# kdexd/virtex

Measured on NVIDIA H100. Metric: image-caption pairs/sec bicaptioning R50-L1-H1024, higher is better.
Workload: dtype bf16

## Files before the change

virtex_b200/csrc/gemm_tc.cu:

```cuda
#include <stdlib.h>
#include "ptx.cuh"
#include "vtx_common.cuh"
#include "../../include/virtex_b200.h"

#define KP_TAPS_W p.taps_w
#define KP_PAD p.pad
#define KP_NTAPS p.ntaps

namespace vtx {

constexpr int kBM = 128;
constexpr int kBK = 64;
constexpr int kMaxStages = 8;
constexpr int kABytes = kBM * kBK * 2;
constexpr int kSmemTotal = 232448;
constexpr int kCtrlBytes = 1024;
constexpr int kThreads = 384;
constexpr int kEpiThreads = 256;

struct FastDiv {
  uint32_t mul, shr;
};
__device__ __forceinline__ int fdiv(int x, const FastDiv& f) {
  return f.mul == 0u ? x : (int)(__umulhi((uint32_t)x, f.mul) >> f.shr);
// ... 684 lines not shown
      }
      if (bnr_on) {
        const uint32_t cp = smem_u32(cbuf) + (scg >> 3) * 16384 + bnr_r0 * 128;
        const int c8 = scg & 7;
        float mean[8], sc[8], sh[8];
        {
          const float4 m0 = __ldg(reinterpret_cast<const float4*>(p.bnr_bnp + bnr_col));
          const float4 m1 = __ldg(reinterpret_cast<const float4*>(p.bnr_bnp + bnr_col + 4));
          mean[0] = m0.x; mean[1] = m0.y; mean[2] = m0.z; mean[3] = m0.w;
          mean[4] = m1.x; mean[5] = m1.y; mean[6] = m1.z; mean[7] = m1.w;
          const float4 a0 = __ldg(reinterpret_cast<const float4*>(p.bnr_bnp + 2 * p.N + bnr_col));
          const float4 a1 = __ldg(reinterpret_cast<const float4*>(p.bnr_bnp + 2 * p.N + bnr_col + 4));
          const float4 b0 = __ldg(reinterpret_cast<const float4*>(p.bnr_bnp + 3 * p.N + bnr_col));
          const float4 b1 = __ldg(reinterpret_cast<const float4*>(p.bnr_bnp + 3 * p.N + bnr_col + 4));
          sc[0] = a0.x; sc[1] = a0.y; sc[2] = a0.z; sc[3] = a0.w; sc[4] = a1.x; sc[5] = a1.y; sc[6] = a1.z; sc[7] = a1.w;
          sh[0] = b0.x; sh[1] = b0.y; sh[2] = b0.z; sh[3] = b0.w; sh[4] = b1.x; sh[5] = b1.y; sh[6] = b1.z; sh[7] = b1.w;
        }
        for (int rb = 0; rb < st_rpt; rb += 4) {
          uint4 yv[4];
          uint32_t mbits;
          bnr_load(rb, yv, mbits);
#pragma unroll
          for (int r4 = 0; r4 < 4; ++r4) {
            const int r = rb + r4;
            const uint4 raw = lds128(cp + r * 128 + ((c8 ^ ((bnr_r0 + r) & 7)) << 4));
            float f[8], yy[8];
            unpack8(*reinterpret_cast<const bf16x8*>(&raw), f);
            unpack8(*reinterpret_cast<const bf16x8*>(&yv[r4]), yy);
#pragma unroll
            for (int i = 0; i < 8; ++i) {
              const bool on = p.bnr == 1 ? ((yy[i] * sc[i] + sh[i] > 0.f) && ((mbits >> (8 * r4)) & 0xffu) != 0u)
                                         : (((mbits >> (8 * r4 + i)) & 1u) != 0u);
              const float dz = on ? f[i] : 0.f;
              st_s[i] += dz;
              st_q[i] += dz * (yy[i] - mean[i]);
            }
          }
        }
      }
      if (!p.bnr && p.stats != nullptr && st_on) {
        const int r0 = srg * st_rpt;
        const uint32_t cp = smem_u32(cbuf) + (scg >> 3) * 16384 + r0 * 128;
        const int c8 = scg & 7;
        for (int rb = 0; rb < st_rpt; rb += 4) {
#pragma unroll
          for (int r4 = 0; r4 < 4; ++r4) {
            const int r = rb + r4;
            const uint4 raw = lds128(cp + r * 128 + ((c8 ^ ((r0 + r) & 7)) << 4));
            float f[8];
            unpack8(*reinterpret_cast<const bf16x8*>(&raw), f);
#pragma unroll
            for (int i = 0; i < 8; ++i) {
              st_s[i] += f[i];
              st_q[i] += f[i] * f[i];
            }
          }
        }
      }
    }
  }
  if (staged) {
    if (et == 0) tma_store_wait_read<0>();
    epi_bar(bar_id, epi_threads);
    if (p.stats != nullptr && st_nt >= 0) flush_stats(cstage0 + (PP ? (size_t)wg * p.cbytes : 0));
  }
}

typedef CUresult (*PFN_encodeTiled)(CUtensorMap*, CUtensorMapDataType, cuuint32_t, void*, const cuuint64_t*,
                                    const cuuint64_t*, const cuuint32_t*, const cuuint32_t*, CUtensorMapInterleave,
                                    CUtensorMapSwizzle, CUtensorMapL2promotion, CUtensorMapFloatOOBfill);

static PFN_encodeTiled get_encode() {
  static PFN_encodeTiled fn = nullptr;
  if (fn == nullptr) {
    void* p = nullptr;
    cudaDriverEntryPointQueryResult q;
    if (cudaGetDriverEntryPoint("cuTensorMapEncodeTiled", &p, cudaEnableDefault, &q) == cudaSuccess &&
        q == cudaDriverEntryPointSuccess)
      fn = reinterpret_cast<PFN_encodeTiled>(p);
  }
  return fn;
}

static int make_tmap(CUtensorMap* tm, const void* ptr, int rank, const uint64_t* dims, const uint64_t* strides_elems,
                     const uint32_t* box, const uint32_t* estr = nullptr) {
  PFN_encodeTiled enc = get_encode();
  if (!enc) return set_error(VTX_ECUDA, "cuTensorMapEncodeTiled entry point not available");
  cuuint64_t gdim[5];
  cuuint64_t gstr[5];
  cuuint32_t bx[5];
  cuuint32_t es[5];
  for (int i = 0; i < rank; ++i) {
    gdim[i] = dims[i];
    bx[i] = box[i];
    es[i] = estr ? estr[i] : 1;
  }
  for (int i = 0; i < rank - 1; ++i) gstr[i] = strides_elems[i] * 2;
  if ((reinterpret_cast<uintptr_t>(ptr) & 15) != 0) return set_error(VTX_EINVAL, "TMA base pointer not 16B aligned");
  for (int i = 0; i < rank - 1; ++i)
    if (gstr[i] % 16 != 0) return set_error(VTX_EINVAL, "TMA stride not a multiple of 16 bytes");
  CUresult r = enc(tm, CU_TENSOR_MAP_DATA_TYPE_BFLOAT16, (cuuint32_t)rank, const_cast<void*>(ptr), gdim, gstr, bx, es,
                   CU_TENSOR_MAP_INTERLEAVE_NONE, CU_TENSOR_MAP_SWIZZLE_128B, CU_TENSOR_MAP_L2_PROMOTION_L2_256B,
                   CU_TENSOR_MAP_FLOAT_OOB_FILL_NONE);
  if (r != CUDA_SUCCESS) return set_error(VTX_ECUDA, "cuTensorMapEncodeTiled failed (%d)", (int)r);
  return VTX_OK;
}

constexpr int kSchedSlots = 4096;
static int g_sched_dynamic = 0;
static struct SchedRing {
  unsigned int* ctr;
  unsigned int base[kSchedSlots];
  unsigned int next;
} g_sched[64];
static bool sched_is_dynamic() {
  static const char* env = getenv("VTX_GEMM_SCHEDULE");
  return env != nullptr ? (env[0] == 'd') : (g_sched_dynamic != 0);
}
static unsigned int* sched_slot(unsigned int fetches, unsigned int* base_out) {
  if (!sched_is_dynamic()) return nullptr;
  int dev = 0;
  cudaGetDevice(&dev);
  if (dev < 0 || dev >= 64) return nullptr;
  SchedRing& r = g_sched[dev];
  if (r.ctr == nullptr) {
    unsigned int* ptr = nullptr;
    if (cudaMalloc(&ptr, sizeof(unsigned int) * kSchedSlots) != cudaSuccess) return nullptr;
    cudaMemset(ptr, 0, sizeof(unsigned int) * kSchedSlots);
    cudaDeviceSynchronize();
    memset(r.base, 0, sizeof(r.base));
    r.next = 0;
    r.ctr = ptr;
  }
  const unsigned int slot = r.next++ % kSchedSlots;
  *base_out = r.base[slot];
  r.base[slot] += fetches;
  return r.ctr + slot;
}

static int ilog2(int x) {
  int l = 0;
  while ((1 << l) < x) ++l;
  return l;
}

static void choose_box(int H, int W, int positions, int* bw, int* bh, int* bn) {
  int best_w = 1, best_h = 1;
  double best_eff = -1;
  for (int w = 1; w <= positions; w <<= 1)
    for (int h = 1; w * h <= positions; h <<= 1) {
      if (w > 2 * W || h > 2 * H) continue;
      const int tw = (W + w - 1) / w, th = (H + h - 1) / h;
      const double eff = (double)(W * H) / ((double)tw * w * th * h);
      const double score = eff * 1000.0 + w * 0.01 + h * 0.0001;
      if (score > best_eff) { best_eff = score; best_w = w; best_h = h; }
    }
  *bw = best_w; *bh = best_h; *bn = positions / (best_w * best_h);
}

template <bool SS>
static cudaError_t launch_gemm(const cudaLaunchConfig_t& cfg, bool pingpong, int bn, const CUtensorMap& tmA,
                               const CUtensorMap& tmB, const CUtensorMap& tmD, const CUtensorMap& tmR,
                               const CUtensorMap& tmY, const GemmKParams& p) {
  if (pingpong && bn == 64) return cudaLaunchKernelEx(&cfg, gemm_wgmma_kernel<64, true, SS>, tmA, tmB, tmD, tmR, tmY, p);
  if (pingpong) return cudaLaunchKernelEx(&cfg, gemm_wgmma_kernel<128, true, SS>, tmA, tmB, tmD, tmR, tmY, p);
  if (bn == 64) return cudaLaunchKernelEx(&cfg, gemm_wgmma_kernel<64, false, SS>, tmA, tmB, tmD, tmR, tmY, p);
  if (bn == 128) return cudaLaunchKernelEx(&cfg, gemm_wgmma_kernel<128, false, SS>, tmA, tmB, tmD, tmR, tmY, p);
  if (bn == 192) return cudaLaunchKernelEx(&cfg, gemm_wgmma_kernel<192, false, SS>, tmA, tmB, tmD, tmR, tmY, p);
  return cudaLaunchKernelEx(&cfg, gemm_wgmma_kernel<256, false, SS>, tmA, tmB, tmD, tmR, tmY, p);
}

bool resid_dgrad_serves(const VtxGemm* g);
int resid_dgrad(const VtxGemm* g, cudaStream_t stream);

}

using namespace vtx;

extern "C" int vtx_gemm_set_dynamic_schedule(int on) {
  g_sched_dynamic = on ? 1 : 0;
  return VTX_OK;
}

extern "C" int vtx_gemm(const VtxGemm* g, void* stream_) {
  cudaStream_t stream = reinterpret_cast<cudaStream_t>(stream_);
  if (!g || !g->A || !g->B || !g->D) return set_error(VTX_EINVAL, "vtx_gemm: null pointer");
  if (g->M <= 0 || g->N <= 0 || g->K <= 0) return set_error(VTX_EINVAL, "vtx_gemm: empty problem");
  if (g->atomic && !g->out_f32) return set_error(VTX_EINVAL, "vtx_gemm: atomic accumulate needs fp32 output");
  if (g->split_k > 1 && !g->atomic) return set_error(VTX_EINVAL, "vtx_gemm: split_k > 1 needs atomic = 1");
  if (g->stats && (g->out_f32 || g->bias || g->residual || g->act || (g->alpha != 0.f && g->alpha != 1.f)))
    return set_error(VTX_EINVAL, "vtx_gemm: stats needs a plain bf16 output (no bias/residual/activation/alpha)");
  if (g->ldd % (g->out_f32 ? 4 : 8) != 0) return set_error(VTX_EINVAL, "vtx_gemm: ldd must keep rows 16B aligned");
  if (g->conv_mode < 0 || g->conv_mode > 6 || g->conv_mode == 3)
    return set_error(VTX_EINVAL, "vtx_gemm: conv_mode must be 0, 1, 2, 4, 5 or 6");
  VtxGemm g4;
  const bool trans_d = g->conv_mode == 4;
  if (trans_d) {
    if (g->conv_c != 64 || g->N != 64 || g->M != 9 * 64 || !g->out_f32 || !g->atomic)
      return set_error(VTX_EINVAL, "vtx_gemm: conv_mode 4 needs C = Cout = 64, M = 576, fp32 atomic output");
    g4 = *g;
    g4.conv_mode = 2;
    g4.M = g->N;
    g4.N = g->M;
    g4.split_k = vtx_num_sms() / 3;
    g4.conv_stride = 1;
    g4.conv_taps = 0;
    g = &g4;
  }
  const int split_k = g->split_k > 1 ? g->split_k : 1;

  GemmKParams p;
  memset(&p, 0, sizeof(p));
  p.M = g->M; p.N = g->N; p.K = g->K;
  p.a_mn = g->a_mn; p.b_mn = g->b_mn;
  p.mode = g->conv_mode;
  const bool stem = g->conv_mode == 5 || g->conv_mode == 6;
  p.taps_w = 3; p.pad = 1; p.ntaps = 9;
  if (stem) { p.mode = g->conv_mode == 5 ? 1 : 2; p.taps_w = 1; p.pad = 0; p.ntaps = 4; }
  const bool one_tap = !stem && g->conv_taps == 1;
  if (one_tap) { p.taps_w = 1; p.pad = 0; p.ntaps = 1; }
  const bool tap_grid = !stem && !one_tap && g->conv_taps_h > 0;
  if (tap_grid) {
    if (p.mode != 1 || g->conv_taps_w <= 0 || g->conv_taps_h > 3 || g->conv_taps_w > 3 || g->conv_pad < 0 || g->conv_pad > 1)
      return set_error(VTX_EINVAL, "vtx_gemm: bad explicit tap grid");
    p.taps_w = g->conv_taps_w; p.pad = g->conv_pad; p.ntaps = g->conv_taps_h * g->conv_taps_w;
  }
  const int cstride = (g->conv_stride == 2 && (p.mode == 1 || p.mode == 2) && !stem) ? 2 : 1;
  if (g->conv_stride != 0 && g->conv_stride != 1 && cstride != 2)
    return set_error(VTX_EINVAL, "vtx_gemm: conv_stride 2 is supported for conv_mode 1 / 2 only");
  if (g->conv_taps != 0 && g->conv_taps != 1 && g->conv_taps != 9) return set_error(VTX_EINVAL, "vtx_gemm: conv_taps must be 0, 1 or 9");
  p.cstride = cstride;
  const int ntaps = stem ? 4 : one_tap ? 1 : tap_grid ? p.ntaps : 9;
  if (p.mode == 1) { p.a_mn = 0; p.b_mn = 0; }
  if (p.mode == 2) { p.a_mn = 1; p.b_mn = 1; }
  int bn = g->tile_n;
  if (bn == 0) {
    const int gran = p.b_mn ? 64 : 16;
    if (g->N >= 256) bn = 256;
    else bn = ((g->N + gran - 1) / gran) * gran;
    if (bn == 256 && split_k == 1) {
      const long mt = (g->M + kBM - 1) / kBM;
      const long t256 = mt * ((g->N + 255) / 256);
      const int sms = vtx_num_sms();
      if (t256 < 100 || (t256 < sms && g->N % 256 != 0 && g->N <= 2048)) {
        bn = 128;
      } else if (t256 < 3L * sms && p.mode <= 1) {
        long best_cost = 0;
        int best_bn = 256;
        for (int cand = 256; cand >= 128; cand -= 64) {
          const long tiles = mt * ((g->N + cand - 1) / cand);
          const long cost = ((tiles + sms - 1) / sms) * (cand + 64);
          if (best_cost == 0 || cost < best_cost) { best_cost = cost; best_bn = cand; }
        }
        bn = best_bn;
      }
    }
  }
  if (bn < 16 || bn > 256 || bn % 16 != 0 || (p.b_mn && bn % 64 != 0))
    return set_error(VTX_EINVAL, "vtx_gemm: bad tile_n %d", bn);
  bn = bn <= 64 ? 64 : bn <= 128 ? 128 : bn <= 192 ? 192 : 256;
  const bool pingpong = bn <= 128 && !g->out_f32;
  p.bn = bn;
  p.n_tiles = (g->N + bn - 1) / bn;
  p.trans_d = trans_d ? 1 : 0;
  p.out_f32 = g->out_f32; p.atomic = g->atomic; p.act = g->act;
  p.alpha = g->alpha == 0.f ? 1.0f : g->alpha;
  p.D = g->D; p.ldd = g->ldd;
  p.bias = g->bias;
  p.bias_pairs = (g->bias != nullptr && g->N % 2 == 0 && (reinterpret_cast<uintptr_t>(g->bias) & 7) == 0) ? 1 : 0;
  p.residual = reinterpret_cast<const __nv_bfloat16*>(g->residual);
  p.ldr = g->ldr;
  const bool mask_rows = g->conv_mode == 0 || (g->conv_mode == 1 && g->conv_out_w <= 0);
  p.res_mask = reinterpret_cast<const uint8_t*>(g->residual_mask);
  if (p.res_mask != nullptr && (g->residual == nullptr || g->N % 32 != 0 || !mask_rows || g->out_f32 ||
                                (reinterpret_cast<uintptr_t>(g->residual_mask) & 3) != 0))
    return set_error(VTX_EINVAL, "vtx_gemm: residual_mask needs a residual, a bf16 output of a plain GEMM or of conv_mode "
                                 "1 without an output view, and N %% 32 == 0");
  p.stats = g->stats;
  const bool bnr = g->bnr_y != nullptr;
  if (bnr) {
    if (!g->bnr_bnp || !g->bnr_sums || g->stats || g->out_f32 || g->bias || g->act || (g->alpha != 0.f && g->alpha != 1.f) ||
        g->N % 8 != 0 || g->bnr_ldy % 8 != 0 || (reinterpret_cast<uintptr_t>(g->bnr_y) & 15) != 0 ||
        (reinterpret_cast<uintptr_t>(g->bnr_bnp) & 15) != 0 || (g->bnr_mask != nullptr && !mask_rows) ||
        g->conv_mode == 2 || g->conv_mode >= 4 || split_k > 1)
      return set_error(VTX_EINVAL, "vtx_gemm: bnr needs a plain bf16 output (no stats/bias/activation/alpha/split-K), "
                                   "N %% 8 == 0, 16-byte aligned y / bnp; the bit-mask form needs conv_mode 0, or 1 without an output view");
    if ((long long)g->M * (g->bnr_ldy > g->N ? g->bnr_ldy : g->N) >= (1ll << 31))
      return set_error(VTX_EUNSUPPORTED, "vtx_gemm: bnr needs M * ld(y) < 2^31");
    p.stats = g->bnr_sums;
    p.bnr_y = reinterpret_cast<const __nv_bfloat16*>(g->bnr_y);
    p.bnr_bnp = g->bnr_bnp;
    p.bnr_mask = g->bnr_mask;
    p.bnr_ldy = g->bnr_ldy;
    const char* pf = getenv("VTX_BNR_PREFETCH");
    p.bnr_prefetch = (pf != nullptr && pf[0] == '0') ? 0 : 1;
    p.bnr = g->bnr_mask == nullptr ? 1 : 2;
  }
  if (g->tile_n == 0 && resid_dgrad_serves(g)) return resid_dgrad(g, stream);
  const bool ss = g->col_scale != nullptr || g->col_shift != nullptr;
  if (ss) {
    if (!g->col_scale || !g->col_shift || g->out_f32 || (g->alpha != 0.f && g->alpha != 1.f) || g->bias || g->stats ||
        bnr || g->act < 0 || g->act > 1 || g->N % 2 != 0 || (reinterpret_cast<uintptr_t>(g->col_scale) & 7) != 0 ||
        (reinterpret_cast<uintptr_t>(g->col_shift) & 7) != 0 || g->residual_mask || g->conv_out_w > 0 ||
        (g->conv_mode != 0 && g->conv_mode != 1) ||
        (g->residual && (g->ldr % 8 != 0 || (reinterpret_cast<uintptr_t>(g->residual) & 15) != 0)))
      return set_error(VTX_EINVAL, "vtx_gemm: col_scale / col_shift need both vectors 8-byte aligned, a bf16 output, "
                                   "alpha 1, act 0 or 1, N %% 2 == 0, conv_mode 0 or 1 without an output view, no bias / "
                                   "stats / bnr / residual mask, and a 16-byte aligned residual with ldr %% 8 == 0");
    p.col_scale = g->col_scale;
    p.col_shift = g->col_shift;
  }

  CUtensorMap tmA, tmB;
  int rc;
  if (p.mode == 0) {
    p.m_tiles = (g->M + kBM - 1) / kBM;
    p.kb_total = (g->K + kBK - 1) / kBK;
    {
      uint64_t dims[2], str[1];
      uint32_t box[2];
      if (!p.a_mn) { dims[0] = g->K; dims[1] = g->M; box[0] = 64; box[1] = 128; }
      else { dims[0] = g->M; dims[1] = g->K; box[0] = 64; box[1] = 64; }
      str[0] = g->lda;
      if ((rc = make_tmap(&tmA, g->A, 2, dims, str, box)) != VTX_OK) return rc;
    }
    {
      uint64_t dims[2], str[1];
      uint32_t box[2];
      if (!p.b_mn) { dims[0] = g->K; dims[1] = g->N; box[0] = 64; box[1] = (uint32_t)bn; }
      else { dims[0] = g->N; dims[1] = g->K; box[0] = 64; box[1] = 64; }
      str[0] = g->ldb;
      if ((rc = make_tmap(&tmB, g->B, 2, dims, str, box)) != VTX_OK) return rc;
    }
  } else {
    const int C = g->conv_c, Hin = g->conv_h, Win = g->conv_w, NI = g->conv_n;
    const int H = (Hin - 1) / cstride + 1, W = (Win - 1) / cstride + 1;
    if (C <= 0 || C % 64 != 0) return set_error(VTX_EINVAL, "vtx_gemm: implicit conv needs channels %% 64 == 0");
    p.cH = H; p.cW = W; p.cN = NI; p.cpb = C / 64;
    const uint64_t xdims[4] = {(uint64_t)C, (uint64_t)Win, (uint64_t)(stem ? Hin + 3 : Hin), (uint64_t)NI};
    const uint64_t xstr[3] = {(uint64_t)(stem ? 16 : C), stem ? (uint64_t)(Win + 3) * 16 : (uint64_t)Win * C,
                              stem ? (uint64_t)(Hin + 3) * (Win + 3) * 16 : (uint64_t)Hin * Win * C};
    int bw, bh, bnn;
    choose_box(H, W, p.mode == 1 ? 128 : 64, &bw, &bh, &bnn);
    p.lbw = ilog2(bw); p.lbh = ilog2(bh); p.lbn = ilog2(bnn);
    p.tiles_w = (W + bw - 1) / bw;
    p.tiles_h = (H + bh - 1) / bh;
    const int tiles_n = (NI + bnn - 1) / bnn;
    if (p.mode == 1) {
      if (g->M != NI * H * W || g->K != ntaps * C) return set_error(VTX_EINVAL, "vtx_gemm: conv fprop shape mismatch");
      if (stem && g->stats && (W % bw != 0 || H % bh != 0))
        return set_error(VTX_EUNSUPPORTED, "vtx_gemm: conv_mode 5 with stats needs an output size tiled exactly by %dx%d", bw, bh);
      p.m_tiles = p.tiles_w * p.tiles_h * tiles_n;
      p.kb_total = ntaps * p.cpb;
      uint32_t box[4] = {64, (uint32_t)(bw * cstride), (uint32_t)(bh * cstride), (uint32_t)bnn};
      const uint32_t es[4] = {1, (uint32_t)cstride, (uint32_t)cstride, 1};
      if ((rc = make_tmap(&tmA, g->A, 4, xdims, xstr, box, cstride > 1 ? es : nullptr)) != VTX_OK) return rc;
      uint64_t bd[2] = {(uint64_t)g->K, (uint64_t)g->N};
      uint64_t bs[1] = {(uint64_t)g->ldb};
      uint32_t bb[2] = {64, (uint32_t)bn};
      if ((rc = make_tmap(&tmB, g->B, 2, bd, bs, bb)) != VTX_OK) return rc;
    } else {
      if (g->N != ntaps * C) return set_error(VTX_EINVAL, "vtx_gemm: conv wgrad shape mismatch");
      const int Cout = g->M;
      if (Cout % 64 != 0) return set_error(VTX_EINVAL, "vtx_gemm: conv wgrad needs Cout %% 64 == 0");
      p.m_tiles = (Cout + kBM - 1) / kBM;
      p.kb_total = p.tiles_w * p.tiles_h * tiles_n;
      uint64_t ad[4] = {(uint64_t)Cout, (uint64_t)W, (uint64_t)H, (uint64_t)NI};
      uint64_t as[3] = {(uint64_t)Cout, (uint64_t)W * Cout, (uint64_t)H * W * Cout};
      uint32_t box[4] = {64, (uint32_t)bw, (uint32_t)bh, (uint32_t)bnn};
      if ((rc = make_tmap(&tmA, g->A, 4, ad, as, box)) != VTX_OK) return rc;
      uint32_t xbox[4] = {64, (uint32_t)(bw * cstride), (uint32_t)(bh * cstride), (uint32_t)bnn};
      const uint32_t es[4] = {1, (uint32_t)cstride, (uint32_t)cstride, 1};
      if ((rc = make_tmap(&tmB, g->B, 4, xdims, xstr, xbox, cstride > 1 ? es : nullptr)) != VTX_OK) return rc;
    }
  }
  p.k_splits = split_k;
  if (p.k_splits > p.kb_total) p.k_splits = p.kb_total;
  p.kb_per_split = (p.kb_total + p.k_splits - 1) / p.k_splits;
  p.k_splits = (p.kb_total + p.kb_per_split - 1) / p.kb_per_split;

  p.stage_bytes = kABytes + bn * kBK * 2;
// ... 117 lines not shown
```

Baseline: 6106.

## Add halo-tiled 3x3 conv kernels for 64-channel forward/dgrad and weight-grad paths

Adds specialized WGMMA kernels for 3x3 convolutions with 64 input and 64 output channels. Each 8x8 spatial tile loads a halo region once through three shifted TMA boxes and reuses it across all nine taps, replacing per-tap implicit-GEMM loads. Weights stay resident in shared memory, and BN-stats and BN-ReLU-backward epilogues are fused in. A separate weight-grad kernel accumulates in registers across tiles and does a single fp32 atomic flush per CTA, instead of split-K through the generic GEMM. Both kernels only apply when H and W are multiples of 8, and they add new code paths that need their own correctness checks.

```diff
diff --git a/virtex_b200/csrc/conv3x3_halo.cu b/virtex_b200/csrc/conv3x3_halo.cu
--- /dev/null
+++ b/virtex_b200/csrc/conv3x3_halo.cu
@@ -0,0 +1,483 @@
+#include "ptx.cuh"
+#include "vtx_common.cuh"
+#include "../../include/virtex_b200.h"
+
+namespace vtx {
+
+int make_tmap(CUtensorMap* tm, const void* ptr, int rank, const uint64_t* dims, const uint64_t* strides_elems,
+              const uint32_t* box, const uint32_t* estr);
+
+namespace {
+
+constexpr int kHMaxStages = 8;
+constexpr int kHThreads = 288;
+constexpr int kHSmem = 232448;
+constexpr int kHCtrl = 1024;
+constexpr int kHBox = 8 * 10 * 128;
+constexpr int kHHalo = 3 * kHBox;
+constexpr int kHTile = 64 * 128;
+constexpr int kHW = 9 * kHTile;
+
+enum { kEpiPlain = 0, kEpiStats = 1, kEpiBnr = 2 };
+
+struct HaloParams {
+  int tiles, tiles_w, tiles_hw;
+  int stages, stage_bytes;
+  const float* bnp;
+  float* sums;
+};
+
+__device__ __forceinline__ uint32_t lds32h(uint32_t a) {
+  uint32_t v;
+  asm volatile("ld.shared.b32 %0, [%1];" : "=r"(v) : "r"(a));
+  return v;
+}
+__device__ __forceinline__ void sts32h(uint32_t a, uint32_t v) {
+  asm volatile("st.shared.b32 [%0], %1;" ::"r"(a), "r"(v) : "memory");
+}
+__device__ __forceinline__ void named_bar_h(int id, int threads) {
+  asm volatile("bar.sync %0, %1;" ::"r"(id), "r"(threads) : "memory");
+}
+
+__device__ __forceinline__ void tile_origin(const HaloParams& p, int tile, int& w0, int& h0, int& n) {
+  n = tile / p.tiles_hw;
+  const int r = tile - n * p.tiles_hw;
+  const int th = r / p.tiles_w;
+  h0 = 8 * th;
+  w0 = 8 * (r - th * p.tiles_w);
+}
+
+template <int EPI>
+__global__ void __launch_bounds__(kHThreads, 1)
+conv3x3_halo_kernel(const __grid_constant__ CUtensorMap tmX, const __grid_constant__ CUtensorMap tmW,
+                    const __grid_constant__ CUtensorMap tmY, const __grid_constant__ CUtensorMap tmD,
+                    const HaloParams p) {
+  VTX_PDL_TRIGGER();
+  extern __shared__ uint8_t smem_raw[];
+  uint8_t* base = reinterpret_cast<uint8_t*>((reinterpret_cast<uintptr_t>(smem_raw) + 1023) & ~uintptr_t(1023));
+  uint64_t* full_bar = reinterpret_cast<uint64_t*>(base);
+  uint64_t* empty_bar = full_bar + kHMaxStages;
+  uint64_t* w_bar = empty_bar + kHMaxStages;
+  float* s_mean = reinterpret_cast<float*>(base + 256);
+  float* s_sc = reinterpret_cast<float*>(base + 512);
+  float* s_sh = reinterpret_cast<float*>(base + 768);
+  uint8_t* sW = base + kHCtrl;
+  uint8_t* sOut = sW + kHW;
+  uint8_t* sStage = sOut + 2 * kHTile;
+
+  const int warp = __shfl_sync(0xffffffffu, (int)(threadIdx.x >> 5), 0);
+  const int lane = threadIdx.x & 31;
+
+  if (warp == 8 && lane == 0) {
+    tma_prefetch_desc(&tmX);
+    tma_prefetch_desc(&tmW);
+    tma_prefetch_desc(&tmD);
+    if (EPI == kEpiBnr) tma_prefetch_desc(&tmY);
+    for (int i = 0; i < p.stages; ++i) {
+      mbar_init(&full_bar[i], 1);
+      mbar_init(&empty_bar[i], 1);
+    }
+    mbar_init(w_bar, 1);
+    fence_mbar_init();
+  }
+  __syncthreads();
+  VTX_PDL_WAIT();
+
+  if (warp == 8) {
+    if (lane == 0) {
+      mbar_arrive_expect_tx(w_bar, (uint32_t)kHW);
+      for (int tap = 0; tap < 9; ++tap) tma_load_2d(sW + tap * kHTile, &tmW, w_bar, tap * 64, 0);
+      const uint32_t tx = (uint32_t)(kHHalo + (EPI == kEpiBnr ? kHTile : 0));
+      int s = 0;
+      for (int tile = blockIdx.x; tile < p.tiles; tile += gridDim.x, ++s) {
+        const int stage = s % p.stages;
+        mbar_wait(&empty_bar[stage], ((uint32_t)(s / p.stages) & 1u) ^ 1u);
+        uint8_t* st = sStage + stage * p.stage_bytes;
+        uint64_t* fb = &full_bar[stage];
+        mbar_arrive_expect_tx(fb, tx);
+        int w0, h0, n;
+        tile_origin(p, tile, w0, h0, n);
+        for (int dw = 0; dw < 3; ++dw) tma_load_4d(st + dw * kHBox, &tmX, fb, 0, w0 + dw - 1, h0 - 1, n);
+        if (EPI == kEpiBnr) tma_load_4d(st + kHHalo, &tmY, fb, 0, w0, h0, n);
+      }
+    }
+    return;
+  }
+
+  const int ct = threadIdx.x;
+  const int wg = ct >> 7;
+  const int wl = (ct >> 5) & 3;
+  const int t = ct & 127;
+  const int q = lane & 3;
+  const int sw = lane >> 2;
+  if (EPI == kEpiBnr) {
+    if (ct < 64) {
+      s_mean[ct] = __ldg(p.bnp + ct);
+      s_sc[ct] = __ldg(p.bnp + 128 + ct);
+      s_sh[ct] = __ldg(p.bnp + 192 + ct);
+    }
+    named_bar_h(3, 256);
+  }
+  constexpr int NP = EPI != kEpiPlain ? 16 : 1;
+  float ps[NP], pq[NP];
+#pragma unroll
+  for (int i = 0; i < NP; ++i) ps[i] = pq[i] = 0.f;
+
+  uint8_t* out = sOut + wg * kHTile;
+  const uint32_t sW0 = smem_u32(sW);
+  mbar_wait(w_bar, 0);
+  for (int s = wg;; s += 2) {
+    const int tile = blockIdx.x + s * gridDim.x;
+    if (tile >= p.tiles) break;
+    const int stage = s % p.stages;
+    const int round = s / p.stages;
+    if (round > 0) mbar_wait(&empty_bar[stage], (uint32_t)(round - 1) & 1u);
+    mbar_wait(&full_bar[stage], (uint32_t)round & 1u);
+    const uint32_t st = smem_u32(sStage + stage * p.stage_bytes);
+
+    float acc[32];
+#pragma unroll
+    for (int i = 0; i < 32; ++i) fence_operand(acc[i]);
+    wgmma_fence();
+#pragma unroll
+    for (int tap = 0; tap < 9; ++tap) {
+      const uint32_t a0 = st + (tap % 3) * kHBox + (tap / 3) * 1024;
+#pragma unroll
+      for (int k = 0; k < 4; ++k) {
+        const uint64_t ad = make_wgmma_desc(a0 + k * 32, 16, 1024);
+        const uint64_t bd = make_wgmma_desc(sW0 + tap * kHTile + k * 32, 16, 1024);
+        wgmma_n64<0, 0>(acc, ad, bd, (tap > 0 || k > 0) ? 1u : 0u);
+      }
+    }
+    wgmma_commit();
+    wgmma_wait<0>();
+#pragma unroll
+    for (int i = 0; i < 32; ++i) fence_operand(acc[i]);
+    if (EPI != kEpiBnr && t == 0) mbar_arrive(&empty_bar[stage]);
+
+    if (t == 0) tma_store_wait_read<0>();
+    named_bar_h(1 + wg, 128);
+
+    const uint32_t row0 = (uint32_t)(wl * 16 + sw) * 128 + q * 4;
+    const uint32_t so = smem_u32(out);
+#pragma unroll
+    for (int j = 0; j < 8; ++j) {
+      const uint32_t off = row0 + (((uint32_t)j ^ sw) << 4);
+      float2 mean = make_float2(0.f, 0.f), sc = mean, sh = mean;
+      if (EPI == kEpiBnr) {
+        mean = *reinterpret_cast<const float2*>(s_mean + 8 * j + 2 * q);
+        sc = *reinterpret_cast<const float2*>(s_sc + 8 * j + 2 * q);
+        sh = *reinterpret_cast<const float2*>(s_sh + 8 * j + 2 * q);
+      }
+#pragma unroll
+      for (int hh = 0; hh < 2; ++hh) {
+        const uint32_t a = off + hh * 8 * 128;
+        const __nv_bfloat162 o2 = __floats2bfloat162_rn(acc[4 * j + 2 * hh], acc[4 * j + 2 * hh + 1]);
+        const uint32_t o = *reinterpret_cast<const uint32_t*>(&o2);
+        sts32h(so + a, o);
+        const float f0 = __uint_as_float(o << 16), f1 = __uint_as_float(o & 0xffff0000u);
+        if (EPI == kEpiStats) {
+          ps[2 * j] += f0;
+          ps[2 * j + 1] += f1;
+          pq[2 * j] += f0 * f0;
+          pq[2 * j + 1] += f1 * f1;
+        } else if (EPI == kEpiBnr) {
+          const uint32_t yw = lds32h(st + kHHalo + a);
+          const float y0 = __uint_as_float(yw << 16), y1 = __uint_as_float(yw & 0xffff0000u);
+          const float dz0 = (y0 * sc.x + sh.x > 0.f) ? f0 : 0.f;
+          const float dz1 = (y1 * sc.y + sh.y > 0.f) ? f1 : 0.f;
+          ps[2 * j] += dz0;
+          ps[2 * j + 1] += dz1;
+          pq[2 * j] += dz0 * (y0 - mean.x);
+          pq[2 * j + 1] += dz1 * (y1 - mean.y);
+        }
+      }
+    }
+    fence_proxy_async();
+    named_bar_h(1 + wg, 128);
+    if (t == 0) {
+      if (EPI == kEpiBnr) mbar_arrive(&empty_bar[stage]);
+      int w0, h0, n;
+      tile_origin(p, tile, w0, h0, n);
+      tma_store_4d(&tmD, out, 0, w0, h0, n);
+      tma_store_commit();
+    }
+  }
+  if (t == 0) tma_store_wait_read<0>();
+  if (EPI != kEpiPlain) {
+#pragma unroll
+    for (int i = 0; i < NP; ++i) {
+#pragma unroll
+      for (int o = 4; o < 32; o <<= 1) {
+        ps[i] += __shfl_xor_sync(0xffffffffu, ps[i], o);
+        pq[i] += __shfl_xor_sync(0xffffffffu, pq[i], o);
+      }
+    }
+    named_bar_h(3, 256);
+    float2* scr = reinterpret_cast<float2*>(sOut);
+    if (sw == 0) {
+#pragma unroll
+      for (int j = 0; j < 8; ++j) {
+        scr[warp * 64 + 8 * j + 2 * q] = make_float2(ps[2 * j], pq[2 * j]);
+        scr[warp * 64 + 8 * j + 2 * q + 1] = make_float2(ps[2 * j + 1], pq[2 * j + 1]);
+      }
+    }
+    named_bar_h(3, 256);
+    if (ct < 64) {
+      float a = 0.f, b = 0.f;
+      for (int w = 0; w < 8; ++w) {
+        const float2 v = scr[w * 64 + ct];
+        a += v.x;
+        b += v.y;
+      }
+      if (EPI == kEpiBnr) b *= __ldg(p.bnp + 64 + ct);
+      atomicAdd(p.sums + ct, a);
+      atomicAdd(p.sums + 64 + ct, b);
+    }
+  }
+}
+
+constexpr int kGThreads = 416;
+constexpr int kGStage = kHHalo + kHTile;
+
+struct WgradParams {
+  int tiles, tiles_w, tiles_hw;
+  int stages;
+  float alpha;
+  float* D;
+  long long ldd;
+};
+
+__global__ void __launch_bounds__(kGThreads, 1)
+conv3x3_halo_wgrad_kernel(const __grid_constant__ CUtensorMap tmX, const __grid_constant__ CUtensorMap tmDy,
+                          const WgradParams p) {
+  VTX_PDL_TRIGGER();
+  extern __shared__ uint8_t smem_raw[];
+  uint8_t* base = reinterpret_cast<uint8_t*>((reinterpret_cast<uintptr_t>(smem_raw) + 1023) & ~uintptr_t(1023));
+  uint64_t* full_bar = reinterpret_cast<uint64_t*>(base);
+  uint64_t* empty_bar = full_bar + kHMaxStages;
+  uint8_t* sStage = base + kHCtrl;
+  HaloParams tp;
+  tp.tiles_w = p.tiles_w;
+  tp.tiles_hw = p.tiles_hw;
+
+  const int warp = __shfl_sync(0xffffffffu, (int)(threadIdx.x >> 5), 0);
+  const int lane = threadIdx.x & 31;
+  if (warp == 12 && lane == 0) {
+    tma_prefetch_desc(&tmX);
+    tma_prefetch_desc(&tmDy);
+    for (int i = 0; i < p.stages; ++i) {
+      mbar_init(&full_bar[i], 1);
+      mbar_init(&empty_bar[i], 3);
+    }
+    fence_mbar_init();
+  }
+  __syncthreads();
+  VTX_PDL_WAIT();
+
+  if (warp == 12) {
+    if (lane == 0) {
+      int s = 0;
+      for (int tile = blockIdx.x; tile < p.tiles; tile += gridDim.x, ++s) {
+        const int stage = s % p.stages;
+        mbar_wait(&empty_bar[stage], ((uint32_t)(s / p.stages) & 1u) ^ 1u);
+        uint8_t* st = sStage + stage * kGStage;
+        uint64_t* fb = &full_bar[stage];
+        mbar_arrive_expect_tx(fb, (uint32_t)kGStage);
+        int w0, h0, n;
+        tile_origin(tp, tile, w0, h0, n);
+        for (int dw = 0; dw < 3; ++dw) tma_load_4d(st + dw * kHBox, &tmX, fb, 0, w0 + dw - 1, h0 - 1, n);
+        tma_load_4d(st + kHHalo, &tmDy, fb, 0, w0, h0, n);
+      }
+    }
+    return;
+  }
+
+  const int dh = threadIdx.x >> 7;
+  const int wl = (threadIdx.x >> 5) & 3;
+  const bool signal = (threadIdx.x & 127) == 0;
+  float acc[96];
+#pragma unroll
+  for (int i = 0; i < 96; ++i) acc[i] = 0.f;
+  int prev = -1;
+  int s = 0;
+  for (int tile = blockIdx.x; tile < p.tiles; tile += gridDim.x, ++s) {
+    const int stage = s % p.stages;
+    mbar_wait(&full_bar[stage], (uint32_t)(s / p.stages) & 1u);
+    const uint32_t st = smem_u32(sStage + stage * kGStage);
+#pragma unroll
+    for (int i = 0; i < 96; ++i) fence_operand(acc[i]);
+    wgmma_fence();
+#pragma unroll
+    for (int k = 0; k < 4; ++k) {
+      const uint64_t ad = make_wgmma_desc(st + kHHalo + k * 2048, 8192, 1024);
+      const uint64_t bd = make_wgmma_desc(st + (2 * k + dh) * 1024, kHBox, 1024);
+      wgmma_n192<1, 1>(acc, ad, bd, 1u);
+    }
+    wgmma_commit();
+    wgmma_wait<1>();
+#pragma unroll
+    for (int i = 0; i < 96; ++i) fence_operand(acc[i]);
+    if (prev >= 0 && signal) mbar_arrive(&empty_bar[prev]);
+    prev = stage;
+  }
+  wgmma_wait<0>();
+#pragma unroll
+  for (int i = 0; i < 96; ++i) fence_operand(acc[i]);
+
+  const int q = lane & 3;
+#pragma unroll
+  for (int hh = 0; hh < 2; ++hh) {
+    const int n = wl * 16 + (lane >> 2) + 8 * hh;
+#pragma unroll
+    for (int j = 0; j < 24; ++j) {
+      const int row = (dh * 3 + (j >> 3)) * 64 + 8 * (j & 7) + 2 * q;
+      float* op = p.D + (long long)row * p.ldd + n;
+      atomicAdd(op, acc[4 * j + 2 * hh] * p.alpha);
+      atomicAdd(op + p.ldd, acc[4 * j + 2 * hh + 1] * p.alpha);
+    }
+  }
+}
+
+template <int EPI>
+cudaError_t launch_halo(const cudaLaunchConfig_t& cfg, const CUtensorMap& tmX, const CUtensorMap& tmW,
+                        const CUtensorMap& tmY, const CUtensorMap& tmD, const HaloParams& p) {
+  cudaError_t e = cudaFuncSetAttribute(conv3x3_halo_kernel<EPI>, cudaFuncAttributeMaxDynamicSharedMemorySize, kHSmem);
+  if (e != cudaSuccess) return e;
+  return cudaLaunchKernelEx(&cfg, conv3x3_halo_kernel<EPI>, tmX, tmW, tmY, tmD, p);
+}
+
+bool al16h(const void* p) { return (reinterpret_cast<uintptr_t>(p) & 15) == 0; }
+
+int halo_stage_bytes(const VtxGemm* g) { return kHHalo + (g->bnr_y != nullptr ? kHTile : 0); }
+int halo_stages(const VtxGemm* g) {
+  const int st = (kHSmem - 1024  - kHCtrl - kHW - 2 * kHTile) / halo_stage_bytes(g);
+  return st > kHMaxStages ? kHMaxStages : st;
+}
+
+}
+
+bool conv3x3_halo_serves(const VtxGemm* g) {
+  const bool bnr = g->bnr_y != nullptr;
+  if (g->conv_mode != 1 || g->conv_c != 64 || g->N != 64 || g->K != 9 * 64 || (g->conv_stride != 0 && g->conv_stride != 1) ||
+      (g->conv_taps != 0 && g->conv_taps != 9) || g->conv_taps_h > 0 || g->conv_out_w > 0)
+    return false;
+  if (g->conv_n <= 0 || g->conv_h <= 0 || g->conv_w <= 0 || g->conv_h % 8 || g->conv_w % 8 ||
+      g->M != g->conv_n * g->conv_h * g->conv_w)
+    return false;
+  if (g->out_f32 || g->atomic || g->split_k > 1 || g->act || g->bias || g->residual || g->residual_mask ||
+      (g->alpha != 0.f && g->alpha != 1.f) || g->col_scale || g->col_shift)
+    return false;
+  if (g->ldb % 8 || g->ldd % 8 || !al16h(g->A) || !al16h(g->B) || !al16h(g->D)) return false;
+  if (bnr && (g->bnr_mask || !g->bnr_bnp || !g->bnr_sums || g->bnr_ldy % 8 || !al16h(g->bnr_y))) return false;
+  return true;
+}
+
+int conv3x3_halo(const VtxGemm* g, cudaStream_t stream) {
+  const bool bnr = g->bnr_y != nullptr;
+  const uint64_t NI = (uint64_t)g->conv_n, H = (uint64_t)g->conv_h, W = (uint64_t)g->conv_w;
+  CUtensorMap tmX, tmW, tmY, tmD;
+  memset(&tmY, 0, sizeof(tmY));
+  int rc;
+  {
+    const uint64_t dims[4] = {64, W, H, NI}, str[3] = {64, W * 64, H * W * 64};
+    const uint32_t box[4] = {64, 8, 10, 1};
+    if ((rc = make_tmap(&tmX, g->A, 4, dims, str, box, nullptr)) != VTX_OK) return rc;
+  }
+  {
+    const uint64_t dims[2] = {9 * 64, 64}, str[1] = {(uint64_t)g->ldb};
+    const uint32_t box[2] = {64, 64};
+    if ((rc = make_tmap(&tmW, g->B, 2, dims, str, box, nullptr)) != VTX_OK) return rc;
+  }
+  const uint32_t tbox[4] = {64, 8, 8, 1};
+  {
+    const uint64_t ld = (uint64_t)g->ldd;
+    const uint64_t dims[4] = {64, W, H, NI}, str[3] = {ld, W * ld, H * W * ld};
+    if ((rc = make_tmap(&tmD, g->D, 4, dims, str, tbox, nullptr)) != VTX_OK) return rc;
+  }
+  if (bnr) {
+    const uint64_t ld = (uint64_t)g->bnr_ldy;
+    const uint64_t dims[4] = {64, W, H, NI}, str[3] = {ld, W * ld, H * W * ld};
+    if ((rc = make_tmap(&tmY, g->bnr_y, 4, dims, str, tbox, nullptr)) != VTX_OK) return rc;
+  }
+  HaloParams p;
+  memset(&p, 0, sizeof(p));
+  p.tiles_w = (int)(W / 8);
+  p.tiles_hw = p.tiles_w * (int)(H / 8);
+  p.tiles = p.tiles_hw * (int)NI;
+  p.stage_bytes = halo_stage_bytes(g);
+  p.stages = halo_stages(g);
+  p.bnp = g->bnr_bnp;
+  p.sums = bnr ? g->bnr_sums : g->stats;
+  const int sms = vtx_num_sms();
+  cudaLaunchConfig_t cfg;
+  memset(&cfg, 0, sizeof(cfg));
+  cfg.gridDim = dim3((unsigned)(p.tiles < sms ? p.tiles : sms));
+  cfg.blockDim = dim3(kHThreads);
+  cfg.dynamicSmemBytes = kHSmem;
+  cfg.stream = stream;
+  cudaLaunchAttribute attr[1];
+  attr[0].id = cudaLaunchAttributeProgrammaticStreamSerialization;
+  attr[0].val.programmaticStreamSerializationAllowed = 1;
+  cfg.attrs = attr;
+  cfg.numAttrs = 1;
+  const cudaError_t le = bnr ? launch_halo<kEpiBnr>(cfg, tmX, tmW, tmY, tmD, p)
+                         : g->stats ? launch_halo<kEpiStats>(cfg, tmX, tmW, tmY, tmD, p)
+                                    : launch_halo<kEpiPlain>(cfg, tmX, tmW, tmY, tmD, p);
+  if (le != cudaSuccess) return set_error(VTX_ECUDA, "conv3x3_halo_kernel launch: %s", cudaGetErrorString(le));
+  return VTX_OK;
+}
+
+
+bool conv3x3_halo_wgrad_serves(const VtxGemm* g) {
+  if (g->conv_mode != 4 || g->conv_c != 64 || g->N != 64 || g->M != 9 * 64 || !g->out_f32 || !g->atomic)
+    return false;
+  if (g->conv_n <= 0 || g->conv_h <= 0 || g->conv_w <= 0 || g->conv_h % 8 || g->conv_w % 8 ||
+      g->K != g->conv_n * g->conv_h * g->conv_w)
+    return false;
+  if ((g->alpha != 0.f && g->alpha != 1.f) || g->ldd < 64 || !al16h(g->A) || !al16h(g->B)) return false;
+  return true;
+}
+
+int conv3x3_halo_wgrad(const VtxGemm* g, cudaStream_t stream) {
+  const uint64_t NI = (uint64_t)g->conv_n, H = (uint64_t)g->conv_h, W = (uint64_t)g->conv_w;
+  CUtensorMap tmX, tmDy;
+  int rc;
+  const uint64_t dims[4] = {64, W, H, NI}, str[3] = {64, W * 64, H * W * 64};
+  {
+    const uint32_t box[4] = {64, 8, 10, 1};
+    if ((rc = make_tmap(&tmX, g->B, 4, dims, str, box, nullptr)) != VTX_OK) return rc;
+  }
+  {
+    const uint32_t box[4] = {64, 8, 8, 1};
+    if ((rc = make_tmap(&tmDy, g->A, 4, dims, str, box, nullptr)) != VTX_OK) return rc;
+  }
+  WgradParams p;
+  memset(&p, 0, sizeof(p));
+  p.tiles_w = (int)(W / 8);
+  p.tiles_hw = p.tiles_w * (int)(H / 8);
+  p.tiles = p.tiles_hw * (int)NI;
+  const int st = (kHSmem - 1024  - kHCtrl) / kGStage;
+  p.stages = st > kHMaxStages ? kHMaxStages : st;
+  p.alpha = 1.f;
+  p.D = reinterpret_cast<float*>(g->D);
+  p.ldd = g->ldd;
+  const int sms = vtx_num_sms();
+  cudaLaunchConfig_t cfg;
+  memset(&cfg, 0, sizeof(cfg));
+  cfg.gridDim = dim3((unsigned)(p.tiles < sms ? p.tiles : sms));
+  cfg.blockDim = dim3(kGThreads);
+  cfg.dynamicSmemBytes = kHSmem;
+  cfg.stream = stream;
+  cudaLaunchAttribute attr[1];
+  attr[0].id = cudaLaunchAttributeProgrammaticStreamSerialization;
+  attr[0].val.programmaticStreamSerializationAllowed = 1;
+  cfg.attrs = attr;
+  cfg.numAttrs = 1;
+  cudaError_t le = cudaFuncSetAttribute(conv3x3_halo_wgrad_kernel, cudaFuncAttributeMaxDynamicSharedMemorySize, kHSmem);
+  if (le == cudaSuccess) le = cudaLaunchKernelEx(&cfg, conv3x3_halo_wgrad_kernel, tmX, tmDy, p);
+  if (le != cudaSuccess) return set_error(VTX_ECUDA, "conv3x3_halo_wgrad_kernel launch: %s", cudaGetErrorString(le));
+  return VTX_OK;
+}
+
+}
diff --git a/virtex_b200/csrc/gemm_tc.cu b/virtex_b200/csrc/gemm_tc.cu
--- a/virtex_b200/csrc/gemm_tc.cu
+++ b/virtex_b200/csrc/gemm_tc.cu
@@ -790,8 +790,8 @@
   return fn;
 }
 
-static int make_tmap(CUtensorMap* tm, const void* ptr, int rank, const uint64_t* dims, const uint64_t* strides_elems,
-                     const uint32_t* box, const uint32_t* estr = nullptr) {
+int make_tmap(CUtensorMap* tm, const void* ptr, int rank, const uint64_t* dims, const uint64_t* strides_elems,
+              const uint32_t* box, const uint32_t* estr = nullptr) {
   PFN_encodeTiled enc = get_encode();
   if (!enc) return set_error(VTX_ECUDA, "cuTensorMapEncodeTiled entry point not available");
   cuuint64_t gdim[5];
@@ -880,6 +880,10 @@
 
 bool resid_dgrad_serves(const VtxGemm* g);
 int resid_dgrad(const VtxGemm* g, cudaStream_t stream);
+bool conv3x3_halo_serves(const VtxGemm* g);
+int conv3x3_halo(const VtxGemm* g, cudaStream_t stream);
+bool conv3x3_halo_wgrad_serves(const VtxGemm* g);
+int conv3x3_halo_wgrad(const VtxGemm* g, cudaStream_t stream);
 
 }
 
@@ -906,6 +910,7 @@
   if (trans_d) {
     if (g->conv_c != 64 || g->N != 64 || g->M != 9 * 64 || !g->out_f32 || !g->atomic)
       return set_error(VTX_EINVAL, "vtx_gemm: conv_mode 4 needs C = Cout = 64, M = 576, fp32 atomic output");
+    if (g->tile_n == 0 && conv3x3_halo_wgrad_serves(g)) return conv3x3_halo_wgrad(g, stream);
     g4 = *g;
     g4.conv_mode = 2;
     g4.M = g->N;
@@ -1005,6 +1010,7 @@
     p.bnr = g->bnr_mask == nullptr ? 1 : 2;
   }
   if (g->tile_n == 0 && resid_dgrad_serves(g)) return resid_dgrad(g, stream);
+  if (g->tile_n == 0 && conv3x3_halo_serves(g)) return conv3x3_halo(g, stream);
   const bool ss = g->col_scale != nullptr || g->col_shift != nullptr;
   if (ss) {
     if (!g->col_scale || !g->col_shift || g->out_f32 || (g->alpha != 0.f && g->alpha != 1.f) || g->bias || g->stats ||
```

Measured after the change: 6288 (median of 6 runs). +3.0%, better.

## Add specialized halo-tiled implicit-GEMM kernel for 64-channel 3x3 convolutions

Applied to the files above, without the earlier changes.

Adds a dedicated WGMMA kernel for 3x3 stride-1 convolutions with 64 input and 64 output channels, the layer1 shape in ResNet-50. The kernel keeps all nine weight taps resident in shared memory and loads one 10x10 halo tile per pair of images with a single TMA. Each tap is then read as a shifted view of that halo, which avoids building the im2col operand tap by tap. The kernel supports plain, batch-norm-stats and BN-ReLU-backward epilogues, with a producer warp and two consumer warpgroups running a multi-stage pipeline. It only serves tightly constrained shapes (H and W multiples of 8, no bias or activation), and adds a second code path that must stay numerically consistent with the general GEMM.

```diff
diff --git a/virtex_b200/csrc/gemm_conv3x3.cu b/virtex_b200/csrc/gemm_conv3x3.cu
--- /dev/null
+++ b/virtex_b200/csrc/gemm_conv3x3.cu
@@ -0,0 +1,332 @@
+#include "ptx.cuh"
+#include "vtx_common.cuh"
+#include "../../include/virtex_b200.h"
+
+namespace vtx {
+
+int make_tmap(CUtensorMap* tm, const void* ptr, int rank, const uint64_t* dims, const uint64_t* strides_elems,
+              const uint32_t* box, const uint32_t* estr = nullptr);
+
+namespace {
+
+constexpr int kCStages = 4;
+constexpr int kCThreads = 288;
+constexpr int kCSmem = 232448;
+constexpr int kCCtrl = 1024;
+constexpr int kHaloW = 10;
+constexpr int kImgBytes = kHaloW * kHaloW * 128;
+constexpr int kHaloBytes = 2 * kImgBytes;
+constexpr int kWBytes = 9 * 64 * 128;
+constexpr int kOutBytes = 128 * 128;
+
+enum { kPlain = 0, kStats = 1, kBnr = 2 };
+
+struct Conv3x3Params {
+  int tiles, tiles_w, tiles_h;
+  float* sums;
+  const float* bnp;
+};
+
+__device__ __forceinline__ uint64_t halo_desc(uint32_t saddr) { return make_wgmma_desc(saddr, 16, kHaloW * 128); }
+__device__ __forceinline__ void bar_named(int id, int threads) {
+  asm volatile("bar.sync %0, %1;" ::"r"(id), "r"(threads) : "memory");
+}
+__device__ __forceinline__ uint32_t lds32c(uint32_t a) {
+  uint32_t v;
+  asm volatile("ld.shared.b32 %0, [%1];" : "=r"(v) : "r"(a));
+  return v;
+}
+__device__ __forceinline__ void sts32c(uint32_t a, uint32_t v) {
+  asm volatile("st.shared.b32 [%0], %1;" ::"r"(a), "r"(v) : "memory");
+}
+__device__ __forceinline__ uint32_t pack_bf16x2_c(float lo, float hi) {
+  const __nv_bfloat162 h = __floats2bfloat162_rn(lo, hi);
+  return *reinterpret_cast<const uint32_t*>(&h);
+}
+__device__ __forceinline__ void tile_origin(const Conv3x3Params& p, int t, int& w0, int& h0, int& n0) {
+  const int r = t / p.tiles_w;
+  const int tn = r / p.tiles_h;
+  w0 = (t - r * p.tiles_w) * 8;
+  h0 = (r - tn * p.tiles_h) * 8;
+  n0 = tn * 2;
+}
+
+template <int EPI>
+__global__ void __launch_bounds__(kCThreads, 1)
+conv3x3_kernel(const __grid_constant__ CUtensorMap tmX, const __grid_constant__ CUtensorMap tmW,
+               const __grid_constant__ CUtensorMap tmY, const __grid_constant__ CUtensorMap tmD,
+               const Conv3x3Params p) {
+  static_assert(kCStages % 2 == 0, "a stage's previous round must belong to the same warpgroup");
+  VTX_PDL_TRIGGER();
+  extern __shared__ uint8_t smem_raw[];
+  uint8_t* base = reinterpret_cast<uint8_t*>((reinterpret_cast<uintptr_t>(smem_raw) + 1023) & ~uintptr_t(1023));
+  uint64_t* full_bar = reinterpret_cast<uint64_t*>(base);
+  uint64_t* empty_bar = full_bar + kCStages;
+  uint64_t* w_bar = empty_bar + kCStages;
+  uint64_t* y_bar = w_bar + 1;
+  float* s_bnp = reinterpret_cast<float*>(base + 256);
+  uint8_t* sW = base + kCCtrl;
+  uint8_t* sOut = sW + kWBytes;
+  uint8_t* sHalo = sOut + 2 * kOutBytes;
+
+  const int warp = __shfl_sync(0xffffffffu, (int)(threadIdx.x >> 5), 0);
+  const int lane = threadIdx.x & 31;
+
+  if (warp == 8 && lane == 0) {
+    tma_prefetch_desc(&tmX);
+    tma_prefetch_desc(&tmW);
+    tma_prefetch_desc(&tmD);
+    if (EPI == kBnr) tma_prefetch_desc(&tmY);
+    for (int i = 0; i < kCStages; ++i) {
+      mbar_init(&full_bar[i], 1);
+      mbar_init(&empty_bar[i], 1);
+    }
+    mbar_init(w_bar, 1);
+    mbar_init(&y_bar[0], 1);
+    mbar_init(&y_bar[1], 1);
+    fence_mbar_init();
+  }
+  __syncthreads();
+  VTX_PDL_WAIT();
+
+  if (warp == 8) {
+    if (lane == 0) {
+      mbar_arrive_expect_tx(w_bar, (uint32_t)kWBytes);
+      for (int tap = 0; tap < 9; ++tap) tma_load_2d(sW + tap * 8192, &tmW, w_bar, tap * 64, 0);
+      int s = 0;
+      for (int t = blockIdx.x; t < p.tiles; t += gridDim.x, ++s) {
+        const int stage = s % kCStages;
+        mbar_wait(&empty_bar[stage], ((uint32_t)(s / kCStages) & 1u) ^ 1u);
+        int w0, h0, n0;
+        tile_origin(p, t, w0, h0, n0);
+        mbar_arrive_expect_tx(&full_bar[stage], (uint32_t)kHaloBytes);
+        tma_load_4d(sHalo + stage * kHaloBytes, &tmX, &full_bar[stage], 0, w0 - 1, h0 - 1, n0);
+      }
+    }
+    return;
+  }
+
+  const int ct = threadIdx.x;
+  const int wg = ct >> 7;
+  const int wl = (ct >> 5) & 3;
+  const bool leader = (ct & 127) == 0;
+  const int q = lane & 3;
+  const int sw = lane >> 2;
+  if (EPI == kBnr) {
+    if (ct < 64) {
+      s_bnp[ct] = __ldg(p.bnp + ct);
+      s_bnp[64 + ct] = __ldg(p.bnp + 128 + ct);
+      s_bnp[128 + ct] = __ldg(p.bnp + 192 + ct);
+    }
+    bar_named(3, 256);
+  }
+  float ps[16], pq[16];
+#pragma unroll
+  for (int i = 0; i < 16; ++i) ps[i] = pq[i] = 0.f;
+
+  uint8_t* out = sOut + wg * kOutBytes;
+  const uint32_t so = smem_u32(out);
+  const uint32_t sw0 = smem_u32(sW);
+  mbar_wait(w_bar, 0);
+  for (int i = wg;; i += 2) {
+    const int t = blockIdx.x + i * gridDim.x;
+    if (t >= p.tiles) break;
+    const int stage = i % kCStages;
+    int w0, h0, n0;
+    tile_origin(p, t, w0, h0, n0);
+    if (leader) {
+      tma_store_wait_read<0>();
+      if (EPI == kBnr) {
+        mbar_arrive_expect_tx(&y_bar[wg], (uint32_t)kOutBytes);
+        tma_load_4d(out, &tmY, &y_bar[wg], 0, w0, h0, n0);
+      }
+    }
+    mbar_wait(&full_bar[stage], (uint32_t)(i / kCStages) & 1u);
+
+    float acc[64];
+#pragma unroll
+    for (int k = 0; k < 64; ++k) fence_operand(acc[k]);
+    const uint32_t halo = smem_u32(sHalo + stage * kHaloBytes);
+    wgmma_fence();
+#pragma unroll
+    for (int tap = 0; tap < 9; ++tap) {
+#pragma unroll
+      for (int k = 0; k < 4; ++k) {
+        const uint64_t bd = make_wgmma_desc(sw0 + tap * 8192 + k * 32, 16, 1024);
+        const uint32_t a0 = halo + ((tap / 3) * kHaloW + tap % 3) * 128 + k * 32;
+#pragma unroll
+        for (int h = 0; h < 2; ++h)
+          wgmma_n64<0, 0>(acc + 32 * h, halo_desc(a0 + h * kImgBytes), bd, (tap > 0 || k > 0) ? 1u : 0u);
+      }
+    }
+    wgmma_commit();
+    wgmma_wait<0>();
+#pragma unroll
+    for (int k = 0; k < 64; ++k) fence_operand(acc[k]);
+    if (EPI == kBnr) mbar_wait(&y_bar[wg], (uint32_t)(i >> 1) & 1u);
+    bar_named(1 + wg, 128);
+    if (leader) mbar_arrive(&empty_bar[stage]);
+
+    const uint32_t row0 = so + (uint32_t)(wl * 16 + sw) * 128 + q * 4;
+#pragma unroll
+    for (int j = 0; j < 8; ++j) {
+      const uint32_t col_off = row0 + (((uint32_t)j ^ (uint32_t)sw) << 4);
+      float2 mean = make_float2(0.f, 0.f), sc = mean, sh = mean;
+      if (EPI == kBnr) {
+        mean = *reinterpret_cast<const float2*>(s_bnp + 8 * j + 2 * q);
+        sc = *reinterpret_cast<const float2*>(s_bnp + 64 + 8 * j + 2 * q);
+        sh = *reinterpret_cast<const float2*>(s_bnp + 128 + 8 * j + 2 * q);
+      }
+#pragma unroll
+      for (int hh = 0; hh < 4; ++hh) {
+        const uint32_t a = col_off + ((hh >> 1) * 64 + 8 * (hh & 1)) * 128;
+        const float* ac = acc + 32 * (hh >> 1) + 4 * j + 2 * (hh & 1);
+        const uint32_t o = pack_bf16x2_c(ac[0], ac[1]);
+        if (EPI != kPlain) {
+          const float d0 = __uint_as_float(o << 16), d1 = __uint_as_float(o & 0xffff0000u);
+          if (EPI == kStats) {
+            ps[2 * j] += d0;
+            ps[2 * j + 1] += d1;
+            pq[2 * j] += d0 * d0;
+            pq[2 * j + 1] += d1 * d1;
+          } else {
+            const uint32_t y = lds32c(a);
+            const float y0 = __uint_as_float(y << 16), y1 = __uint_as_float(y & 0xffff0000u);
+            const float dz0 = (y0 * sc.x + sh.x > 0.f) ? d0 : 0.f;
+            const float dz1 = (y1 * sc.y + sh.y > 0.f) ? d1 : 0.f;
+            ps[2 * j] += dz0;
+            ps[2 * j + 1] += dz1;
+            pq[2 * j] += dz0 * (y0 - mean.x);
+            pq[2 * j + 1] += dz1 * (y1 - mean.y);
+          }
+        }
+        sts32c(a, o);
+      }
+    }
+    fence_proxy_async();
+    bar_named(1 + wg, 128);
+    if (leader) {
+      tma_store_4d(&tmD, out, 0, w0, h0, n0);
+      tma_store_commit();
+    }
+  }
+  if (leader) tma_store_wait_read<0>();
+  if (EPI != kPlain) {
+#pragma unroll
+    for (int k = 0; k < 16; ++k) {
+#pragma unroll
+      for (int o = 4; o < 32; o <<= 1) {
+        ps[k] += __shfl_xor_sync(0xffffffffu, ps[k], o);
+        pq[k] += __shfl_xor_sync(0xffffffffu, pq[k], o);
+      }
+    }
+    bar_named(3, 256);
+    float2* scr = reinterpret_cast<float2*>(sW);
+    if (sw == 0) {
+#pragma unroll
+      for (int j = 0; j < 8; ++j) {
+        scr[warp * 64 + 8 * j + 2 * q] = make_float2(ps[2 * j], pq[2 * j]);
+        scr[warp * 64 + 8 * j + 2 * q + 1] = make_float2(ps[2 * j + 1], pq[2 * j + 1]);
+      }
+    }
+    bar_named(3, 256);
+    if (ct < 64) {
+      float a = 0.f, b = 0.f;
+      for (int w = 0; w < 8; ++w) {
+        const float2 v = scr[w * 64 + ct];
+        a += v.x;
+        b += v.y;
+      }
+      if (EPI == kBnr) b *= __ldg(p.bnp + 64 + ct);
+      atomicAdd(p.sums + ct, a);
+      atomicAdd(p.sums + 64 + ct, b);
+    }
+  }
+}
+
+template <int EPI>
+cudaError_t launch_conv3x3(const cudaLaunchConfig_t& cfg, const CUtensorMap& tmX, const CUtensorMap& tmW,
+                           const CUtensorMap& tmY, const CUtensorMap& tmD, const Conv3x3Params& p) {
+  const cudaError_t e =
+      cudaFuncSetAttribute(conv3x3_kernel<EPI>, cudaFuncAttributeMaxDynamicSharedMemorySize, kCSmem);
+  if (e != cudaSuccess) return e;
+  return cudaLaunchKernelEx(&cfg, conv3x3_kernel<EPI>, tmX, tmW, tmY, tmD, p);
+}
+
+bool al16c(const void* ptr) { return (reinterpret_cast<uintptr_t>(ptr) & 15) == 0; }
+
+}
+
+static_assert(1024 + kCCtrl + kWBytes + 2 * kOutBytes + kCStages * kHaloBytes <= kCSmem, "shared memory");
+
+bool conv3x3_serves(const VtxGemm* g) {
+  if (g->conv_mode != 1 || (g->conv_stride != 0 && g->conv_stride != 1) || (g->conv_taps != 0 && g->conv_taps != 9) ||
+      g->conv_taps_h > 0 || g->conv_out_w > 0)
+    return false;
+  if (g->conv_c != 64 || g->N != 64 || g->K != 9 * 64 || g->conv_h % 8 != 0 || g->conv_w % 8 != 0 || g->conv_h <= 0 ||
+      g->conv_w <= 0 || g->conv_n <= 0 || (long long)g->M != (long long)g->conv_n * g->conv_h * g->conv_w)
+    return false;
+  if (g->out_f32 || g->atomic || g->split_k > 1 || g->act || g->bias || g->residual || g->residual_mask ||
+      (g->alpha != 0.f && g->alpha != 1.f) || g->col_scale || g->col_shift)
+    return false;
+  if (g->stats && g->bnr_y) return false;
+  if (g->bnr_y && (g->bnr_mask || !g->bnr_bnp || !g->bnr_sums || g->bnr_ldy % 8 != 0 || !al16c(g->bnr_y)))
+    return false;
+  return al16c(g->A) && al16c(g->B) && al16c(g->D) && g->ldb % 8 == 0 && g->ldd % 8 == 0;
+}
+
+int conv3x3(const VtxGemm* g, cudaStream_t stream) {
+  const int NI = g->conv_n, H = g->conv_h, W = g->conv_w;
+  const int epi = g->bnr_y ? kBnr : g->stats ? kStats : kPlain;
+  CUtensorMap tmX, tmW, tmY, tmD;
+  memset(&tmY, 0, sizeof(tmY));
+  int rc;
+  {
+    const uint64_t dims[4] = {64, (uint64_t)W, (uint64_t)H, (uint64_t)NI};
+    const uint64_t str[3] = {64, (uint64_t)W * 64, (uint64_t)H * W * 64};
+    const uint32_t box[4] = {64, kHaloW, kHaloW, 2};
+    if ((rc = make_tmap(&tmX, g->A, 4, dims, str, box)) != VTX_OK) return rc;
+  }
+  {
+    const uint64_t dims[2] = {9 * 64, 64};
+    const uint64_t str[1] = {(uint64_t)g->ldb};
+    const uint32_t box[2] = {64, 64};
+    if ((rc = make_tmap(&tmW, g->B, 2, dims, str, box)) != VTX_OK) return rc;
+  }
+  {
+    const uint64_t dims[4] = {64, (uint64_t)W, (uint64_t)H, (uint64_t)NI};
+    const uint32_t box[4] = {64, 8, 8, 2};
+    const uint64_t ds[3] = {(uint64_t)g->ldd, (uint64_t)W * g->ldd, (uint64_t)H * W * g->ldd};
+    if ((rc = make_tmap(&tmD, g->D, 4, dims, ds, box)) != VTX_OK) return rc;
+    if (epi == kBnr) {
+      const uint64_t ys[3] = {(uint64_t)g->bnr_ldy, (uint64_t)W * g->bnr_ldy, (uint64_t)H * W * g->bnr_ldy};
+      if ((rc = make_tmap(&tmY, g->bnr_y, 4, dims, ys, box)) != VTX_OK) return rc;
+    }
+  }
+  Conv3x3Params p;
+  memset(&p, 0, sizeof(p));
+  p.tiles_w = W / 8;
+  p.tiles_h = H / 8;
+  p.tiles = p.tiles_w * p.tiles_h * ((NI + 1) / 2);
+  p.sums = epi == kBnr ? g->bnr_sums : g->stats;
+  p.bnp = g->bnr_bnp;
+  const int sms = vtx_num_sms();
+  cudaLaunchConfig_t cfg;
+  memset(&cfg, 0, sizeof(cfg));
+  cfg.gridDim = dim3((unsigned)(p.tiles < sms ? p.tiles : sms));
+  cfg.blockDim = dim3(kCThreads);
+  cfg.dynamicSmemBytes = kCSmem;
+  cfg.stream = stream;
+  cudaLaunchAttribute attr[1];
+  attr[0].id = cudaLaunchAttributeProgrammaticStreamSerialization;
+  attr[0].val.programmaticStreamSerializationAllowed = 1;
+  cfg.attrs = attr;
+  cfg.numAttrs = 1;
+  const cudaError_t le = epi == kBnr ? launch_conv3x3<kBnr>(cfg, tmX, tmW, tmY, tmD, p)
+                         : epi == kStats ? launch_conv3x3<kStats>(cfg, tmX, tmW, tmY, tmD, p)
+                                         : launch_conv3x3<kPlain>(cfg, tmX, tmW, tmY, tmD, p);
+  if (le != cudaSuccess) return set_error(VTX_ECUDA, "conv3x3_kernel launch: %s", cudaGetErrorString(le));
+  return VTX_OK;
+}
+
+}
diff --git a/virtex_b200/csrc/gemm_tc.cu b/virtex_b200/csrc/gemm_tc.cu
--- a/virtex_b200/csrc/gemm_tc.cu
+++ b/virtex_b200/csrc/gemm_tc.cu
@@ -790,8 +790,8 @@
   return fn;
 }
 
-static int make_tmap(CUtensorMap* tm, const void* ptr, int rank, const uint64_t* dims, const uint64_t* strides_elems,
-                     const uint32_t* box, const uint32_t* estr = nullptr) {
+int make_tmap(CUtensorMap* tm, const void* ptr, int rank, const uint64_t* dims, const uint64_t* strides_elems,
+              const uint32_t* box, const uint32_t* estr = nullptr) {
   PFN_encodeTiled enc = get_encode();
   if (!enc) return set_error(VTX_ECUDA, "cuTensorMapEncodeTiled entry point not available");
   cuuint64_t gdim[5];
@@ -880,6 +880,8 @@
 
 bool resid_dgrad_serves(const VtxGemm* g);
 int resid_dgrad(const VtxGemm* g, cudaStream_t stream);
+bool conv3x3_serves(const VtxGemm* g);
+int conv3x3(const VtxGemm* g, cudaStream_t stream);
 
 }
 
@@ -1005,6 +1007,7 @@
     p.bnr = g->bnr_mask == nullptr ? 1 : 2;
   }
   if (g->tile_n == 0 && resid_dgrad_serves(g)) return resid_dgrad(g, stream);
+  if (g->tile_n == 0 && conv3x3_serves(g)) return conv3x3(g, stream);
   const bool ss = g->col_scale != nullptr || g->col_shift != nullptr;
   if (ss) {
     if (!g->col_scale || !g->col_shift || g->out_f32 || (g->alpha != 0.f && g->alpha != 1.f) || g->bias || g->stats ||
```

Result: faster. 6098 before, 6199 after, median of 6 (+1.7%).
